# pythoncrazy/jimm

Measured on NVIDIA H100. Metric: images/sec, higher is better.
Workload: dtype f16

## Files before the change

jimm_b200/csrc/common.cuh:

```cuda
#pragma once

#include <cuda.h>
#include <cuda_bf16.h>
#include <cuda_fp16.h>
#include <cuda_runtime.h>
#include <stdint.h>

namespace jimm {

void set_last_error(const char* fmt, ...);

#define JIMM_CUDA_CHECK(expr)                                                                   \
  do {                                                                                          \
    cudaError_t _e = (expr);                                                                    \
    if (_e != cudaSuccess) {                                                                    \
      ::jimm::set_last_error("%s:%d: %s -> %s", __FILE__, __LINE__, #expr, cudaGetErrorString(_e)); \
      return -2;                                                                                \
    }                                                                                           \
  } while (0)

void note_launch();
#define JIMM_LAUNCH_CHECK()                  \
  do {                                       \
    JIMM_CUDA_CHECK(cudaGetLastError());     \
    ::jimm::note_launch();                   \
  } while (0)

int pdl_enabled();
template <typename... KArgs, typename... Args>
inline cudaError_t launch_k(void (*kernel)(KArgs...), dim3 grid, dim3 block, size_t smem, cudaStream_t stream, int cluster_x, bool pdl,
                            Args&&... args) {
  cudaLaunchConfig_t cfg = {};
  cfg.gridDim = grid;
  cfg.blockDim = block;
  cfg.dynamicSmemBytes = smem;
  cfg.stream = stream;
  cudaLaunchAttribute attr[2];
  unsigned n = 0;
  if (pdl && pdl_enabled()) {
    attr[n].id = cudaLaunchAttributeProgrammaticStreamSerialization;
    attr[n].val.programmaticStreamSerializationAllowed = 1;
    ++n;
  }
  if (cluster_x > 1) {
    attr[n].id = cudaLaunchAttributeClusterDimension;
    attr[n].val.clusterDim.x = static_cast<unsigned>(cluster_x);
    attr[n].val.clusterDim.y = 1;
    attr[n].val.clusterDim.z = 1;
    ++n;
  }
  cfg.attrs = attr;
  cfg.numAttrs = n;
  return cudaLaunchKernelEx(&cfg, kernel, static_cast<KArgs>(args)...);
}

struct DeviceOnce {
  static constexpr int kMaxDevices = 64;
  bool done[kMaxDevices] = {};
  bool first() {
    int dev = 0;
    cudaGetDevice(&dev);
    if (dev < 0 || dev >= kMaxDevices) return true;
    if (done[dev]) return false;
    done[dev] = true;
    return true;
  }
};

__device__ __forceinline__ void pdl_launch_dependents() { asm volatile("griddepcontrol.launch_dependents;" ::: "memory"); }
__device__ __forceinline__ void pdl_wait() { asm volatile("griddepcontrol.wait;" ::: "memory"); }

__device__ __forceinline__ uint32_t smem_u32(const void* p) {
  return static_cast<uint32_t>(__cvta_generic_to_shared(p));
}

__device__ __forceinline__ uint32_t lane_id() {
  uint32_t l;
  asm volatile("mov.u32 %0, %%laneid;" : "=r"(l));
  return l;
}

__device__ __forceinline__ bool elect_one_sync() {
  uint32_t pred = 0;
  asm volatile(
      "{\n\t.reg .pred P1;\n\t"
      "elect.sync _|P1, 0xffffffff;\n\t"
      "selp.u32 %0, 1, 0, P1;\n\t}"
      : "=r"(pred));
  return pred != 0;
}

__device__ __forceinline__ void mbar_init(uint64_t* bar, uint32_t count) {
  asm volatile("mbarrier.init.shared::cta.b64 [%0], %1;" ::"r"(smem_u32(bar)), "r"(count));
}
__device__ __forceinline__ void fence_barrier_init() {
  asm volatile("fence.mbarrier_init.release.cluster;" ::: "memory");
}
__device__ __forceinline__ void fence_proxy_async_smem() {
  asm volatile("fence.proxy.async.shared::cta;" ::: "memory");
}
__device__ __forceinline__ void mbar_arrive(uint64_t* bar) {
  asm volatile("mbarrier.arrive.shared::cta.b64 _, [%0];" ::"r"(smem_u32(bar)) : "memory");
}
__device__ __forceinline__ void mbar_arrive_expect_tx(uint64_t* bar, uint32_t bytes) {
  asm volatile("mbarrier.arrive.expect_tx.shared::cta.b64 _, [%0], %1;" ::"r"(smem_u32(bar)), "r"(bytes) : "memory");
}
__device__ __forceinline__ void mbar_wait(uint64_t* bar, uint32_t parity) {
  asm volatile(
      "{\n\t.reg .pred P1;\n\t"
      "WAIT_LOOP:\n\t"
      "mbarrier.try_wait.parity.shared::cta.b64 P1, [%0], %1;\n\t"
      "@P1 bra DONE;\n\t"
      "bra WAIT_LOOP;\n\t"
      "DONE:\n\t}" ::"r"(smem_u32(bar)),
      "r"(parity)
      : "memory");
}

__device__ __forceinline__ bool mbar_test_wait(uint64_t* bar, uint32_t parity) {
  uint32_t ok;
  asm volatile(
      "{\n\t.reg .pred P1;\n\t"
      "mbarrier.test_wait.parity.shared::cta.b64 P1, [%1], %2;\n\t"
      "selp.u32 %0, 1, 0, P1;\n\t}"
      : "=r"(ok)
      : "r"(smem_u32(bar)), "r"(parity)
      : "memory");
  return ok != 0;
}

__device__ __forceinline__ void tma_prefetch_desc(const CUtensorMap* m) {
  asm volatile("prefetch.tensormap [%0];" ::"l"(reinterpret_cast<uint64_t>(m)) : "memory");
}
__device__ __forceinline__ void tma_load_2d(void* smem_dst, const CUtensorMap* m, uint64_t* bar, int c0, int c1) {
  asm volatile(
      "cp.async.bulk.tensor.2d.shared::cluster.global.mbarrier::complete_tx::bytes [%0], [%1, {%3, %4}], [%2];" ::"r"(
          smem_u32(smem_dst)),
      "l"(reinterpret_cast<uint64_t>(m)), "r"(smem_u32(bar)), "r"(c0), "r"(c1)
      : "memory");
}

__device__ __forceinline__ void tma_store_2d(const CUtensorMap* m, uint32_t smem_src, int c0, int c1) {
  asm volatile("cp.async.bulk.tensor.2d.global.shared::cta.bulk_group [%0, {%2, %3}], [%1];" ::"l"(reinterpret_cast<uint64_t>(m)),
               "r"(smem_src), "r"(c0), "r"(c1)
               : "memory");
}
__device__ __forceinline__ void tma_reduce_add_2d(const CUtensorMap* m, uint32_t smem_src, int c0, int c1) {
  asm volatile("cp.reduce.async.bulk.tensor.2d.global.shared::cta.add.tile.bulk_group [%0, {%2, %3}], [%1];" ::"l"(
                   reinterpret_cast<uint64_t>(m)),
               "r"(smem_src), "r"(c0), "r"(c1)
               : "memory");
}
__device__ __forceinline__ void tma_store_3d(const CUtensorMap* m, uint32_t smem_src, int c0, int c1, int c2) {
  asm volatile("cp.async.bulk.tensor.3d.global.shared::cta.bulk_group [%0, {%2, %3, %4}], [%1];" ::"l"(reinterpret_cast<uint64_t>(m)),
               "r"(smem_src), "r"(c0), "r"(c1), "r"(c2)
               : "memory");
}
__device__ __forceinline__ void tma_reduce_add_3d(const CUtensorMap* m, uint32_t smem_src, int c0, int c1, int c2) {
  asm volatile("cp.reduce.async.bulk.tensor.3d.global.shared::cta.add.tile.bulk_group [%0, {%2, %3, %4}], [%1];" ::"l"(
                   reinterpret_cast<uint64_t>(m)),
               "r"(smem_src), "r"(c0), "r"(c1), "r"(c2)
               : "memory");
}
__device__ __forceinline__ void tma_store_commit() { asm volatile("cp.async.bulk.commit_group;" ::: "memory"); }
__device__ __forceinline__ void tma_store_wait_read() { asm volatile("cp.async.bulk.wait_group.read 0;" ::: "memory"); }
__device__ __forceinline__ void tma_store_wait_read1() { asm volatile("cp.async.bulk.wait_group.read 1;" ::: "memory"); }
__device__ __forceinline__ void tma_store_wait_all() { asm volatile("cp.async.bulk.wait_group 0;" ::: "memory"); }

__device__ __forceinline__ uint32_t cluster_ctarank() {
  uint32_t r;
  asm volatile("mov.u32 %0, %%cluster_ctarank;" : "=r"(r));
  return r;
}
__device__ __forceinline__ void cluster_sync_all() {
  asm volatile("barrier.cluster.arrive.release.aligned;\n\tbarrier.cluster.wait.acquire.aligned;" ::: "memory");
}
__device__ __forceinline__ uint32_t mapa_shared(uint32_t local_smem_addr, uint32_t rank) {
  uint32_t r;
  asm volatile("mapa.shared::cluster.u32 %0, %1, %2;" : "=r"(r) : "r"(local_smem_addr), "r"(rank));
  return r;
}
__device__ __forceinline__ void mbar_arrive_cluster(uint32_t cluster_addr) {
  asm volatile("mbarrier.arrive.release.cluster.shared::cluster.b64 _, [%0];" ::"r"(cluster_addr) : "memory");
}
__device__ __forceinline__ uint64_t make_wgmma_desc_sw128(uint32_t smem_addr) {
  uint64_t d = 0;
  d |= static_cast<uint64_t>((smem_addr & 0x3FFFFu) >> 4);
  d |= static_cast<uint64_t>(1) << 16;
  d |= static_cast<uint64_t>(1024 >> 4) << 32;
  d |= static_cast<uint64_t>(1) << 62;
  return d;
}
__device__ __forceinline__ void wgmma_fence() { asm volatile("wgmma.fence.sync.aligned;" ::: "memory"); }
__device__ __forceinline__ void wgmma_commit() { asm volatile("wgmma.commit_group.sync.aligned;" ::: "memory"); }
template <int N>
__device__ __forceinline__ void wgmma_wait() { asm volatile("wgmma.wait_group.sync.aligned %0;" ::"n"(N) : "memory"); }
template <int R>
__device__ __forceinline__ void wgmma_fence_operands(float (&d)[R]) {
#pragma unroll
  for (int i = 0; i < R; ++i) asm volatile("" : "+f"(d[i])::"memory");
}

template <int KIND>
__device__ __forceinline__ void wgmma_m64n128_ss(float (&d)[64], uint64_t adesc, uint64_t bdesc, uint32_t accumulate) {
  if constexpr (KIND == 0) {
    asm volatile(
        "{\n\t.reg .pred p;\n\t"
        "setp.ne.b32 p, %66, 0;\n\t"
        "wgmma.mma_async.sync.aligned.m64n128k16.f32.f16.f16 {%0, %1, %2, %3, %4, %5, %6, %7, %8, %9, %10, %11, %12, %13, %14, %15, %16, %17, %18, %19, %20, %21, %22, %23, %24, %25, %26, %27, %28, %29, %30, %31, %32, %33, %34, %35, %36, %37, %38, %39, %40, %41, %42, %43, %44, %45, %46, %47, %48, %49, %50, %51, %52, %53, %54, %55, %56, %57, %58, %59, %60, %61, %62, %63}, %64, %65, p, 1, 1, 0, 0;\n\t}"
        : "+f"(d[0]), "+f"(d[1]), "+f"(d[2]), "+f"(d[3]), "+f"(d[4]), "+f"(d[5]), "+f"(d[6]), "+f"(d[7]),
          "+f"(d[8]), "+f"(d[9]), "+f"(d[10]), "+f"(d[11]), "+f"(d[12]), "+f"(d[13]), "+f"(d[14]), "+f"(d[15]),
          "+f"(d[16]), "+f"(d[17]), "+f"(d[18]), "+f"(d[19]), "+f"(d[20]), "+f"(d[21]), "+f"(d[22]), "+f"(d[23]),
          "+f"(d[24]), "+f"(d[25]), "+f"(d[26]), "+f"(d[27]), "+f"(d[28]), "+f"(d[29]), "+f"(d[30]), "+f"(d[31]),
          "+f"(d[32]), "+f"(d[33]), "+f"(d[34]), "+f"(d[35]), "+f"(d[36]), "+f"(d[37]), "+f"(d[38]), "+f"(d[39]),
          "+f"(d[40]), "+f"(d[41]), "+f"(d[42]), "+f"(d[43]), "+f"(d[44]), "+f"(d[45]), "+f"(d[46]), "+f"(d[47]),
          "+f"(d[48]), "+f"(d[49]), "+f"(d[50]), "+f"(d[51]), "+f"(d[52]), "+f"(d[53]), "+f"(d[54]), "+f"(d[55]),
          "+f"(d[56]), "+f"(d[57]), "+f"(d[58]), "+f"(d[59]), "+f"(d[60]), "+f"(d[61]), "+f"(d[62]), "+f"(d[63])
        : "l"(adesc), "l"(bdesc), "r"(accumulate));
  } else if constexpr (KIND == 1) {
    asm volatile(
        "{\n\t.reg .pred p;\n\t"
        "setp.ne.b32 p, %66, 0;\n\t"
        "wgmma.mma_async.sync.aligned.m64n128k16.f32.bf16.bf16 {%0, %1, %2, %3, %4, %5, %6, %7, %8, %9, %10, %11, %12, %13, %14, %15, %16, %17, %18, %19, %20, %21, %22, %23, %24, %25, %26, %27, %28, %29, %30, %31, %32, %33, %34, %35, %36, %37, %38, %39, %40, %41, %42, %43, %44, %45, %46, %47, %48, %49, %50, %51, %52, %53, %54, %55, %56, %57, %58, %59, %60, %61, %62, %63}, %64, %65, p, 1, 1, 0, 0;\n\t}"
        : "+f"(d[0]), "+f"(d[1]), "+f"(d[2]), "+f"(d[3]), "+f"(d[4]), "+f"(d[5]), "+f"(d[6]), "+f"(d[7]),
          "+f"(d[8]), "+f"(d[9]), "+f"(d[10]), "+f"(d[11]), "+f"(d[12]), "+f"(d[13]), "+f"(d[14]), "+f"(d[15]),
          "+f"(d[16]), "+f"(d[17]), "+f"(d[18]), "+f"(d[19]), "+f"(d[20]), "+f"(d[21]), "+f"(d[22]), "+f"(d[23]),
          "+f"(d[24]), "+f"(d[25]), "+f"(d[26]), "+f"(d[27]), "+f"(d[28]), "+f"(d[29]), "+f"(d[30]), "+f"(d[31]),
          "+f"(d[32]), "+f"(d[33]), "+f"(d[34]), "+f"(d[35]), "+f"(d[36]), "+f"(d[37]), "+f"(d[38]), "+f"(d[39]),
          "+f"(d[40]), "+f"(d[41]), "+f"(d[42]), "+f"(d[43]), "+f"(d[44]), "+f"(d[45]), "+f"(d[46]), "+f"(d[47]),
          "+f"(d[48]), "+f"(d[49]), "+f"(d[50]), "+f"(d[51]), "+f"(d[52]), "+f"(d[53]), "+f"(d[54]), "+f"(d[55]),
          "+f"(d[56]), "+f"(d[57]), "+f"(d[58]), "+f"(d[59]), "+f"(d[60]), "+f"(d[61]), "+f"(d[62]), "+f"(d[63])
        : "l"(adesc), "l"(bdesc), "r"(accumulate));
  } else {
    asm volatile(
        "{\n\t.reg .pred p;\n\t"
        "setp.ne.b32 p, %66, 0;\n\t"
        "wgmma.mma_async.sync.aligned.m64n128k8.f32.tf32.tf32 {%0, %1, %2, %3, %4, %5, %6, %7, %8, %9, %10, %11, %12, %13, %14, %15, %16, %17, %18, %19, %20, %21, %22, %23, %24, %25, %26, %27, %28, %29, %30, %31, %32, %33, %34, %35, %36, %37, %38, %39, %40, %41, %42, %43, %44, %45, %46, %47, %48, %49, %50, %51, %52, %53, %54, %55, %56, %57, %58, %59, %60, %61, %62, %63}, %64, %65, p, 1, 1;\n\t}"
        : "+f"(d[0]), "+f"(d[1]), "+f"(d[2]), "+f"(d[3]), "+f"(d[4]), "+f"(d[5]), "+f"(d[6]), "+f"(d[7]),
          "+f"(d[8]), "+f"(d[9]), "+f"(d[10]), "+f"(d[11]), "+f"(d[12]), "+f"(d[13]), "+f"(d[14]), "+f"(d[15]),
          "+f"(d[16]), "+f"(d[17]), "+f"(d[18]), "+f"(d[19]), "+f"(d[20]), "+f"(d[21]), "+f"(d[22]), "+f"(d[23]),
          "+f"(d[24]), "+f"(d[25]), "+f"(d[26]), "+f"(d[27]), "+f"(d[28]), "+f"(d[29]), "+f"(d[30]), "+f"(d[31]),
          "+f"(d[32]), "+f"(d[33]), "+f"(d[34]), "+f"(d[35]), "+f"(d[36]), "+f"(d[37]), "+f"(d[38]), "+f"(d[39]),
          "+f"(d[40]), "+f"(d[41]), "+f"(d[42]), "+f"(d[43]), "+f"(d[44]), "+f"(d[45]), "+f"(d[46]), "+f"(d[47]),
          "+f"(d[48]), "+f"(d[49]), "+f"(d[50]), "+f"(d[51]), "+f"(d[52]), "+f"(d[53]), "+f"(d[54]), "+f"(d[55]),
          "+f"(d[56]), "+f"(d[57]), "+f"(d[58]), "+f"(d[59]), "+f"(d[60]), "+f"(d[61]), "+f"(d[62]), "+f"(d[63])
        : "l"(adesc), "l"(bdesc), "r"(accumulate));
  }
}

template <bool BF16>
__device__ __forceinline__ void wgmma_m64n64k16_ss(float (&d)[32], uint64_t adesc, uint64_t bdesc, uint32_t accumulate) {
  if constexpr (BF16) {
    asm volatile(
        "{\n\t.reg .pred p;\n\t"
        "setp.ne.b32 p, %34, 0;\n\t"
        "wgmma.mma_async.sync.aligned.m64n64k16.f32.bf16.bf16 {%0, %1, %2, %3, %4, %5, %6, %7, %8, %9, %10, %11, %12, %13, %14, %15, %16, %17, %18, %19, %20, %21, %22, %23, %24, %25, %26, %27, %28, %29, %30, %31}, %32, %33, p, 1, 1, 0, 0;\n\t}"
        : "+f"(d[0]), "+f"(d[1]), "+f"(d[2]), "+f"(d[3]), "+f"(d[4]), "+f"(d[5]), "+f"(d[6]), "+f"(d[7]),
          "+f"(d[8]), "+f"(d[9]), "+f"(d[10]), "+f"(d[11]), "+f"(d[12]), "+f"(d[13]), "+f"(d[14]), "+f"(d[15]),
          "+f"(d[16]), "+f"(d[17]), "+f"(d[18]), "+f"(d[19]), "+f"(d[20]), "+f"(d[21]), "+f"(d[22]), "+f"(d[23]),
          "+f"(d[24]), "+f"(d[25]), "+f"(d[26]), "+f"(d[27]), "+f"(d[28]), "+f"(d[29]), "+f"(d[30]), "+f"(d[31])
        : "l"(adesc), "l"(bdesc), "r"(accumulate));
  } else {
    asm volatile(
        "{\n\t.reg .pred p;\n\t"
        "setp.ne.b32 p, %34, 0;\n\t"
        "wgmma.mma_async.sync.aligned.m64n64k16.f32.f16.f16 {%0, %1, %2, %3, %4, %5, %6, %7, %8, %9, %10, %11, %12, %13, %14, %15, %16, %17, %18, %19, %20, %21, %22, %23, %24, %25, %26, %27, %28, %29, %30, %31}, %32, %33, p, 1, 1, 0, 0;\n\t}"
        : "+f"(d[0]), "+f"(d[1]), "+f"(d[2]), "+f"(d[3]), "+f"(d[4]), "+f"(d[5]), "+f"(d[6]), "+f"(d[7]),
          "+f"(d[8]), "+f"(d[9]), "+f"(d[10]), "+f"(d[11]), "+f"(d[12]), "+f"(d[13]), "+f"(d[14]), "+f"(d[15]),
          "+f"(d[16]), "+f"(d[17]), "+f"(d[18]), "+f"(d[19]), "+f"(d[20]), "+f"(d[21]), "+f"(d[22]), "+f"(d[23]),
          "+f"(d[24]), "+f"(d[25]), "+f"(d[26]), "+f"(d[27]), "+f"(d[28]), "+f"(d[29]), "+f"(d[30]), "+f"(d[31])
        : "l"(adesc), "l"(bdesc), "r"(accumulate));
  }
}
template <bool BF16>
__device__ __forceinline__ void wgmma_m64n64k16_rs(float (&d)[32], const uint32_t (&a)[4], uint64_t bdesc) {
  if constexpr (BF16) {
    asm volatile(
        "wgmma.mma_async.sync.aligned.m64n64k16.f32.bf16.bf16 {%0, %1, %2, %3, %4, %5, %6, %7, %8, %9, %10, %11, %12, %13, %14, %15, %16, %17, %18, %19, %20, %21, %22, %23, %24, %25, %26, %27, %28, %29, %30, %31}, {%32, %33, %34, %35}, %36, 1, 1, 1, 1;"
        : "+f"(d[0]), "+f"(d[1]), "+f"(d[2]), "+f"(d[3]), "+f"(d[4]), "+f"(d[5]), "+f"(d[6]), "+f"(d[7]),
          "+f"(d[8]), "+f"(d[9]), "+f"(d[10]), "+f"(d[11]), "+f"(d[12]), "+f"(d[13]), "+f"(d[14]), "+f"(d[15]),
          "+f"(d[16]), "+f"(d[17]), "+f"(d[18]), "+f"(d[19]), "+f"(d[20]), "+f"(d[21]), "+f"(d[22]), "+f"(d[23]),
          "+f"(d[24]), "+f"(d[25]), "+f"(d[26]), "+f"(d[27]), "+f"(d[28]), "+f"(d[29]), "+f"(d[30]), "+f"(d[31])
        : "r"(a[0]), "r"(a[1]), "r"(a[2]), "r"(a[3]), "l"(bdesc));
  } else {
    asm volatile(
        "wgmma.mma_async.sync.aligned.m64n64k16.f32.f16.f16 {%0, %1, %2, %3, %4, %5, %6, %7, %8, %9, %10, %11, %12, %13, %14, %15, %16, %17, %18, %19, %20, %21, %22, %23, %24, %25, %26, %27, %28, %29, %30, %31}, {%32, %33, %34, %35}, %36, 1, 1, 1, 1;"
        : "+f"(d[0]), "+f"(d[1]), "+f"(d[2]), "+f"(d[3]), "+f"(d[4]), "+f"(d[5]), "+f"(d[6]), "+f"(d[7]),
          "+f"(d[8]), "+f"(d[9]), "+f"(d[10]), "+f"(d[11]), "+f"(d[12]), "+f"(d[13]), "+f"(d[14]), "+f"(d[15]),
          "+f"(d[16]), "+f"(d[17]), "+f"(d[18]), "+f"(d[19]), "+f"(d[20]), "+f"(d[21]), "+f"(d[22]), "+f"(d[23]),
          "+f"(d[24]), "+f"(d[25]), "+f"(d[26]), "+f"(d[27]), "+f"(d[28]), "+f"(d[29]), "+f"(d[30]), "+f"(d[31])
        : "r"(a[0]), "r"(a[1]), "r"(a[2]), "r"(a[3]), "l"(bdesc));
  }
}

__device__ __forceinline__ void named_bar_sync(int id, int nthreads) { asm volatile("bar.sync %0, %1;" ::"r"(id), "r"(nthreads) : "memory"); }

__device__ __forceinline__ float tanh_fast(float x) {
  float y;
  asm("tanh.approx.f32 %0, %1;" : "=f"(y) : "f"(x));
  return y;
}
__device__ __forceinline__ float ex2_fast(float x) {
  float y;
  asm("ex2.approx.ftz.f32 %0, %1;" : "=f"(y) : "f"(x));
  return y;
}
__device__ __forceinline__ float rcp_fast(float x) {
  float y;
  asm("rcp.approx.ftz.f32 %0, %1;" : "=f"(y) : "f"(x));
  return y;
}
__device__ __forceinline__ float gelu_tanh(float x) {
  const float c0 = -2.0f * 0.7978845608028654f * 1.4426950408889634f;
  const float c1 = c0 * 0.044715f;
  const float z = x * fmaf(x * x, c1, c0);
  return x * rcp_fast(1.0f + ex2_fast(z));
}
__device__ __forceinline__ float quick_gelu(float x) { return x * rcp_fast(1.0f + ex2_fast(x * (-1.702f * 1.4426950408889634f))); }

__device__ __forceinline__ float warp_sum(float v) {
#pragma unroll
  for (int o = 16; o > 0; o >>= 1) v += __shfl_xor_sync(0xffffffffu, v, o);
  return v;
}
__device__ __forceinline__ float warp_max(float v) {
#pragma unroll
  for (int o = 16; o > 0; o >>= 1) v = fmaxf(v, __shfl_xor_sync(0xffffffffu, v, o));
  return v;
}

__device__ __forceinline__ float round_tf32(float v) {
  uint32_t u;
  asm("cvt.rna.tf32.f32 %0, %1;" : "=r"(u) : "f"(v));
  return __uint_as_float(u);
}
struct tf32_t {
  float v;
};

template <typename T>
__device__ __forceinline__ T from_float(float v);
template <>
__device__ __forceinline__ tf32_t from_float<tf32_t>(float v) { return tf32_t{round_tf32(v)}; }
template <>
__device__ __forceinline__ float from_float<float>(float v) { return v; }
template <>
__device__ __forceinline__ __half from_float<__half>(float v) { return __float2half_rn(v); }
template <>
__device__ __forceinline__ __nv_bfloat16 from_float<__nv_bfloat16>(float v) { return __float2bfloat16_rn(v); }

__device__ __forceinline__ float to_float(float v) { return v; }
__device__ __forceinline__ float to_float(__half v) { return __half2float(v); }
__device__ __forceinline__ float to_float(__nv_bfloat16 v) { return __bfloat162float(v); }

__device__ __forceinline__ uint32_t pack2(float a, float b, int out_type ) {
  if (out_type == 1) {
    __half2 h = __floats2half2_rn(a, b);
    return *reinterpret_cast<uint32_t*>(&h);
  } else {
    __nv_bfloat162 h = __floats2bfloat162_rn(a, b);
    return *reinterpret_cast<uint32_t*>(&h);
  }
}

}
```

jimm_b200/csrc/gemm.cu:

```cuda
#include "gemm.cuh"

#include <stdarg.h>
#include <stdio.h>
#include <stdlib.h>
#include <string.h>

#include <type_traits>

#include "common.cuh"

namespace jimm {

static constexpr int BM = 128;
static constexpr int BN = 128;
static constexpr int STAGES = 5;
static constexpr int A_STAGE_BYTES = BM * 128;
static constexpr int B_STAGE_BYTES = BN * 128;
static constexpr int STAGE_BYTES = A_STAGE_BYTES + B_STAGE_BYTES;
static constexpr int EPI_WARPS = 8;
static constexpr int EPI_BOX_ROWS = 16;
static constexpr int EPI_BUF_BYTES = EPI_BOX_ROWS * 128;
static constexpr int EPI_BUFS = 2;
static constexpr int EPI_STAGE_BYTES = EPI_WARPS * EPI_BUFS * EPI_BUF_BYTES;
static constexpr int NUM_THREADS = 384;

enum OutKind : int { OUT_GENERIC = 0, OUT_H16 = 1, OUT_BF16 = 2, OUT_TF32 = 3, OUT_F32_ADD = 4, OUT_F32 = 5 };

struct EpiDev {
  const float* bias;
  const float* rowadd;
  const float* residual;
  void* out;
  int act, ldr, out_type, ldo, rows_in, rows_out, row_off, mode;
  int M, N;
  int reverse;
  int tok_pad, tok_off;
  const float* ln_scale;
  const float* ln_bias;
  void* ln_out;
  int* ln_cnt;
  int ln_out_type, ln_ldo;
  float ln_eps;
};

template <int ACT>
__device__ __forceinline__ float act_ct(float v) {
  if constexpr (ACT == ACT_GELU_TANH) return gelu_tanh(v);
  else if constexpr (ACT == ACT_QUICK_GELU) return quick_gelu(v);
  else return v;
}
__device__ __forceinline__ float apply_act(float v, int act) {
  if (act == ACT_GELU_TANH) return gelu_tanh(v);
  if (act == ACT_QUICK_GELU) return quick_gelu(v);
  return v;
}

__device__ __forceinline__ void remap_row(const EpiDev& e, int row, int& out_row, int& add_row) {
  if (e.rows_in > 0) {
    int b = row / e.rows_in, p = row - b * e.rows_in;
    out_row = b * e.rows_out + p + e.row_off;
    add_row = p + e.row_off;
  } else {
    out_row = row;
    add_row = row;
  }
}

__device__ __forceinline__ void store1(const EpiDev& e, int out_row, int col, float v) {
  size_t off = static_cast<size_t>(out_row) * e.ldo + col;
  if (e.out_type == DT_F32) static_cast<float*>(e.out)[off] = v;
  else if (e.out_type == DT_TF32) static_cast<float*>(e.out)[off] = round_tf32(v);
  else if (e.out_type == DT_F16) static_cast<__half*>(e.out)[off] = __float2half_rn(v);
  else static_cast<__nv_bfloat16*>(e.out)[off] = __float2bfloat16_rn(v);
}

template <typename T>
struct Traits;
template <>
struct Traits<__half> {
  static constexpr int KIND = 0;
};
template <>
struct Traits<__nv_bfloat16> {
  static constexpr int KIND = 1;
};
template <>
struct Traits<float> {
  static constexpr int KIND = 2;
};

static constexpr int ACT_FUSE_LN = 7;
static constexpr int LNQ = 240;
struct LnQueue {
  int head, tail, done, pad;
  int slot[LNQ];
};

template <typename OutT, int NV>
__device__ __forceinline__ void ln_rows_nv(const EpiDev& e, int row0, int lane) {
  constexpr int R0 = 12 / NV;
  constexpr int R = R0 < 1 ? 1 : (R0 > 8 ? 8 : R0);
  constexpr bool DOUBLE = NV <= 9;
  const float inv_d = 1.0f / static_cast<float>(NV * 128);
  const float4* sc = reinterpret_cast<const float4*>(e.ln_scale);
  const float4* bi = reinterpret_cast<const float4*>(e.ln_bias);
  const float* xbase = static_cast<const float*>(e.out);
  const int ldx = e.ldo, ldh = e.ln_ldo;
  const float eps = e.ln_eps;
  OutT* hbase = static_cast<OutT*>(e.ln_out);
  const int rows = min(32, e.M - row0);
  float4 a[R][NV];
  float4 b[DOUBLE ? R : 1][DOUBLE ? NV : 1];
#define JIMM_LN_LOAD(buf, r0_)                                                                                          \
  _Pragma("unroll") for (int i = 0; i < R; ++i) {      \
    const float4* xr = reinterpret_cast<const float4*>(xbase + static_cast<size_t>(row0 + min((r0_) + i, rows - 1)) * ldx); \
    _Pragma("unroll") for (int j = 0; j < NV; ++j) buf[i][j] = __ldcg(xr + lane + 32 * j);                              \
  }
#define JIMM_LN_PROCESS(buf, r0_)                                                                                       \
  _Pragma("unroll") for (int i = 0; i < R; ++i) {                                                                       \
    if ((r0_) + i < rows) {                                                                                             \
      float s = 0.f, s2 = 0.f;                                                                                          \
      _Pragma("unroll") for (int j = 0; j < NV; ++j) {                                                                  \
        const float4 v = buf[i][j];                                                                                     \
        s += v.x + v.y + v.z + v.w;                                                                                     \
        s2 += v.x * v.x + v.y * v.y + v.z * v.z + v.w * v.w;                                                            \
      }                                                                                                                 \
      s = warp_sum(s);                                                                                                  \
      s2 = warp_sum(s2);                                                                                                \
      const float mean = s * inv_d;                                                                                     \
      const float rstd = rsqrtf(fmaxf(s2 * inv_d - mean * mean, 0.0f) + eps);                                           \
      OutT* orow = hbase + static_cast<size_t>(row0 + (r0_) + i) * ldh;                                                 \
      _Pragma("unroll") for (int j = 0; j < NV; ++j) {                                                                  \
        const int idx = lane + 32 * j;                                                                                  \
        const float4 v = buf[i][j], g = __ldg(sc + idx), bb = __ldg(bi + idx);                                          \
        float4 y;                                                                                                       \
        y.x = (v.x - mean) * rstd * g.x + bb.x;                                                                         \
        y.y = (v.y - mean) * rstd * g.y + bb.y;                                                                         \
        y.z = (v.z - mean) * rstd * g.z + bb.z;                                                                         \
        y.w = (v.w - mean) * rstd * g.w + bb.w;                                                                         \
        if constexpr (std::is_same<OutT, float>::value) {                                                               \
          reinterpret_cast<float4*>(orow)[idx] = make_float4(round_tf32(y.x), round_tf32(y.y), round_tf32(y.z), round_tf32(y.w)); \
        } else {                                                                                                        \
          uint2 pk;                                                                                                     \
          constexpr int ot = std::is_same<OutT, __half>::value ? DT_F16 : DT_BF16;                                      \
          pk.x = pack2(y.x, y.y, ot);                                                                                   \
          pk.y = pack2(y.z, y.w, ot);                                                                                   \
          reinterpret_cast<uint2*>(orow)[idx] = pk;                                                                     \
        }                                                                                                               \
      }                                                                                                                 \
    }                                                                                                                   \
  }
  if constexpr (DOUBLE) {
    JIMM_LN_LOAD(a, 0)
#pragma unroll 1
    for (int r0 = 0; r0 < rows; r0 += 2 * R) {
      JIMM_LN_LOAD(b, r0 + R)
      JIMM_LN_PROCESS(a, r0)
      JIMM_LN_LOAD(a, r0 + 2 * R)
      JIMM_LN_PROCESS(b, r0 + R)
    }
  } else {
#pragma unroll 1
    for (int r0 = 0; r0 < rows; r0 += R) {
      JIMM_LN_LOAD(a, r0)
      JIMM_LN_PROCESS(a, r0)
    }
  }
#undef JIMM_LN_LOAD
#undef JIMM_LN_PROCESS
}

template <typename OutT>
__device__ __forceinline__ void ln_rows_dispatch(const EpiDev& e, int row0, int lane) {
  switch (e.N >> 7) {
    case 1: ln_rows_nv<OutT, 1>(e, row0, lane); break;
    case 2: ln_rows_nv<OutT, 2>(e, row0, lane); break;
    case 3: ln_rows_nv<OutT, 3>(e, row0, lane); break;
    case 4: ln_rows_nv<OutT, 4>(e, row0, lane); break;
    case 6: ln_rows_nv<OutT, 6>(e, row0, lane); break;
    case 8: ln_rows_nv<OutT, 8>(e, row0, lane); break;
    case 9: ln_rows_nv<OutT, 9>(e, row0, lane); break;
    case 10: ln_rows_nv<OutT, 10>(e, row0, lane); break;
    case 12: ln_rows_nv<OutT, 12>(e, row0, lane); break;
    default: break;
  }
}

__device__ __forceinline__ void ln_publish(const EpiDev& e, LnQueue* q, int rg, int cols) {
  tma_store_wait_all();
  __threadfence();
  const int old = atomicAdd(e.ln_cnt + rg, cols);
  if (old + cols == 2 * e.N) {
    e.ln_cnt[rg] = 0;
    __threadfence();
    const int t = atomicAdd(&q->tail, 1);
    volatile int* s = &q->slot[t % LNQ];
    while (*s != -1) __nanosleep(64);
    *s = rg;
  }
}

template <typename OutT>
__device__ __forceinline__ void ln_worker(const EpiDev& e, LnQueue* q, int lane) {
  for (;;) {
    int rg = -2;
    if (lane == 0) {
      const int t = atomicAdd(&q->head, 1);
      volatile int* s = &q->slot[t % LNQ];
      for (;;) {
        if (*s >= 0) {
          const int v = atomicExch(&q->slot[t % LNQ], -1);
          if (v >= 0) { rg = v; break; }
        }
        if (*reinterpret_cast<volatile int*>(&q->done) == EPI_WARPS && t >= *reinterpret_cast<volatile int*>(&q->tail)) break;
        __nanosleep(256);
      }
      __threadfence();
    }
    rg = __shfl_sync(0xffffffffu, rg, 0);
    if (rg < 0) return;
    ln_rows_dispatch<OutT>(e, rg * 32, lane);
  }
}

template <int OUT, int ACT>
__device__ __forceinline__ void epilogue_tma(const CUtensorMap* map_c, const EpiDev& epi, const float (&acc)[64], uint8_t* tbuf0, int lane,
                                             int row_base, int n_tile0, uint32_t& box_count) {
  constexpr bool OUT16 = (OUT == OUT_H16 || OUT == OUT_BF16);
  constexpr int ES = OUT16 ? 2 : 4;
  constexpr int COLS_PER_BOX = 128 / ES;
  constexpr int JB = COLS_PER_BOX / 8;
  const int g = lane >> 2, t = lane & 3;
#pragma unroll
  for (int s = 0; s < BN / COLS_PER_BOX; ++s) {
    const int n0 = n_tile0 + s * COLS_PER_BOX;
    if (n0 >= epi.N) break;
    uint8_t* tbuf = tbuf0 + (box_count & (EPI_BUFS - 1)) * EPI_BUF_BYTES;
    ++box_count;
    if (lane == 0) tma_store_wait_read1();
    __syncwarp();
#pragma unroll
    for (int jj = 0; jj < JB; ++jj) {
      const int j = s * JB + jj;
      const int col = n0 + jj * 8 + 2 * t;
      float2 b2 = make_float2(0.f, 0.f);
      if (epi.bias != nullptr && col < epi.N) b2 = __ldg(reinterpret_cast<const float2*>(epi.bias + col));
      const float v0 = act_ct<ACT>(acc[4 * j] + b2.x), v1 = act_ct<ACT>(acc[4 * j + 1] + b2.y);
      const float v2 = act_ct<ACT>(acc[4 * j + 2] + b2.x), v3 = act_ct<ACT>(acc[4 * j + 3] + b2.y);
      const int byte = (jj * 8 + 2 * t) * ES;
      const int off = ((((byte >> 4) ^ g)) << 4) + (byte & 15);
      uint8_t* p0 = tbuf + g * 128 + off;
      uint8_t* p1 = p0 + 8 * 128;
      if constexpr (OUT16) {
        *reinterpret_cast<uint32_t*>(p0) = pack2(v0, v1, OUT == OUT_H16 ? 1 : 2);
        *reinterpret_cast<uint32_t*>(p1) = pack2(v2, v3, OUT == OUT_H16 ? 1 : 2);
      } else if constexpr (OUT == OUT_TF32) {
        *reinterpret_cast<float2*>(p0) = make_float2(round_tf32(v0), round_tf32(v1));
        *reinterpret_cast<float2*>(p1) = make_float2(round_tf32(v2), round_tf32(v3));
      } else {
        *reinterpret_cast<float2*>(p0) = make_float2(v0, v1);
        *reinterpret_cast<float2*>(p1) = make_float2(v2, v3);
      }
    }
    fence_proxy_async_smem();
    __syncwarp();
    if (lane == 0) {
      const uint32_t tbuf_u32 = smem_u32(tbuf);
      if constexpr (OUT == OUT_F32_ADD) {
        if (epi.tok_pad > 0) {
          const int b = row_base / epi.tok_pad;
          tma_reduce_add_3d(map_c, tbuf_u32, n0, row_base - b * epi.tok_pad + epi.tok_off, b);
        } else {
          tma_reduce_add_2d(map_c, tbuf_u32, n0, row_base);
        }
      } else {
        tma_store_2d(map_c, tbuf_u32, n0, row_base);
      }
      tma_store_commit();
    }
  }
}

__device__ __forceinline__ void epilogue_generic(const EpiDev& epi, const float (&acc)[64], int lane, int row_base, int n_tile0) {
  const int g = lane >> 2, t = lane & 3;
#pragma unroll
  for (int h = 0; h < 2; ++h) {
    const int row = row_base + g + 8 * h;
    if (row >= epi.M) continue;
    int out_row, add_row;
    remap_row(epi, row, out_row, add_row);
#pragma unroll
    for (int j = 0; j < BN / 8; ++j) {
#pragma unroll
      for (int q = 0; q < 2; ++q) {
        const int col = n_tile0 + 8 * j + 2 * t + q;
        if (col < epi.N) {
          float v = acc[4 * j + 2 * h + q];
          if (epi.bias) v += __ldg(epi.bias + col);
          v = apply_act(v, epi.act);
          if (epi.rowadd) v += __ldg(epi.rowadd + static_cast<size_t>(add_row) * epi.N + col);
          if (epi.residual) v += epi.residual[static_cast<size_t>(out_row) * epi.ldr + col];
          store1(epi, out_row, col, v);
        }
      }
    }
  }
}

template <typename T, int OUT, int ACT>
__global__ void __launch_bounds__(NUM_THREADS, 1)
gemm_wgmma_kernel(const __grid_constant__ CUtensorMap map_a, const __grid_constant__ CUtensorMap map_b,
                  const __grid_constant__ CUtensorMap map_c, const EpiDev epi, int K) {
  constexpr int BK = 128 / sizeof(T);
  constexpr int UK = 32 / sizeof(T);
  constexpr bool FUSE_LN = OUT == OUT_F32_ADD && ACT == ACT_FUSE_LN;
  constexpr int EPI_ACT = ACT == ACT_FUSE_LN ? static_cast<int>(ACT_NONE) : ACT;

  extern __shared__ uint8_t smem_raw[];
  uint8_t* smem = reinterpret_cast<uint8_t*>((reinterpret_cast<uintptr_t>(smem_raw) + 1023) & ~static_cast<uintptr_t>(1023));
  uint8_t* smem_a = smem;
  uint8_t* smem_b = smem + STAGES * A_STAGE_BYTES;
  uint8_t* epi_stage = smem + STAGES * STAGE_BYTES;
  LnQueue* lnq = reinterpret_cast<LnQueue*>(epi_stage + EPI_STAGE_BYTES);
  uint64_t* full_bar = reinterpret_cast<uint64_t*>(lnq + 1);
  uint64_t* empty_bar = full_bar + STAGES;

  const int warp_idx = threadIdx.x >> 5;
  const int lane = threadIdx.x & 31;
  const int M = epi.M, N = epi.N;
  const int m_tiles = (M + BM - 1) / BM, n_tiles = (N + BN - 1) / BN;
  const int num_tiles = m_tiles * n_tiles;
  const int num_kb = (K + BK - 1) / BK;

  pdl_launch_dependents();
  if (warp_idx == 0 && lane == 0) {
    tma_prefetch_desc(&map_a);
    tma_prefetch_desc(&map_b);
    if constexpr (OUT != OUT_GENERIC) tma_prefetch_desc(&map_c);
    for (int s = 0; s < STAGES; ++s) {
      mbar_init(&full_bar[s], 1);
      mbar_init(&empty_bar[s], EPI_WARPS);
    }
    fence_barrier_init();
  }
  if constexpr (FUSE_LN) {
    if (warp_idx == 1) {
      for (int i = lane; i < LNQ; i += 32) lnq->slot[i] = -1;
      if (lane == 0) lnq->head = lnq->tail = lnq->done = 0;
    }
  }
  __syncthreads();
  pdl_wait();

  if (warp_idx < 4) {
    if (warp_idx == 0) {
      if (lane == 0) {
        int stage = 0;
        uint32_t phase = 0;
        for (int tile = blockIdx.x; tile < num_tiles; tile += gridDim.x) {
          const int tv = epi.reverse ? num_tiles - 1 - tile : tile;
          const int m_blk = tv / n_tiles, n_blk = tv - m_blk * n_tiles;
          for (int kb = 0; kb < num_kb; ++kb) {
            mbar_wait(&empty_bar[stage], phase ^ 1);
            mbar_arrive_expect_tx(&full_bar[stage], STAGE_BYTES);
            tma_load_2d(smem_a + stage * A_STAGE_BYTES, &map_a, &full_bar[stage], kb * BK, m_blk * BM);
            tma_load_2d(smem_b + stage * B_STAGE_BYTES, &map_b, &full_bar[stage], kb * BK, n_blk * BN);
            if (++stage == STAGES) { stage = 0; phase ^= 1; }
          }
        }
      }
    } else if constexpr (FUSE_LN) {
      ln_worker<T>(epi, lnq, lane);
    }
  } else {
    const int wg = (warp_idx - 4) >> 2;
    const int wq = warp_idx & 3;
    uint8_t* tbuf0 = epi_stage + (warp_idx - 4) * EPI_BUFS * EPI_BUF_BYTES;
    int stage = 0;
    uint32_t phase = 0, box_count = 0;
    int ln_rg = -1, ln_cols = 0;
    float acc[64];
    for (int tile = blockIdx.x; tile < num_tiles; tile += gridDim.x) {
      const int tv = epi.reverse ? num_tiles - 1 - tile : tile;
      const int m_blk = tv / n_tiles, n_blk = tv - m_blk * n_tiles;
      int prev = -1;
      for (int kb = 0; kb < num_kb; ++kb) {
        mbar_wait(&full_bar[stage], phase);
        const uint64_t adesc = make_wgmma_desc_sw128(smem_u32(smem_a + stage * A_STAGE_BYTES + wg * 64 * 128));
        const uint64_t bdesc = make_wgmma_desc_sw128(smem_u32(smem_b + stage * B_STAGE_BYTES));
        wgmma_fence_operands(acc);
        wgmma_fence();
#pragma unroll
        for (int k = 0; k < BK / UK; ++k)
          wgmma_m64n128_ss<Traits<T>::KIND>(acc, adesc + static_cast<uint64_t>(2 * k), bdesc + static_cast<uint64_t>(2 * k), (kb | k) != 0 ? 1u : 0u);
        wgmma_commit();
        wgmma_fence_operands(acc);
        if (prev >= 0) {
          wgmma_wait<1>();
          if (lane == 0) mbar_arrive(&empty_bar[prev]);
        }
        prev = stage;
        if (++stage == STAGES) { stage = 0; phase ^= 1; }
      }
      wgmma_wait<0>();
      wgmma_fence_operands(acc);
      if (lane == 0) mbar_arrive(&empty_bar[prev]);

      const int row_base = m_blk * BM + wg * 64 + wq * 16;
      const int n_tile0 = n_blk * BN;
      if constexpr (OUT == OUT_GENERIC) {
        epilogue_generic(epi, acc, lane, row_base, n_tile0);
      } else {
        if (row_base < M) epilogue_tma<OUT, EPI_ACT>(&map_c, epi, acc, tbuf0, lane, row_base, n_tile0, box_count);
        if constexpr (FUSE_LN) {
          if (lane == 0 && ln_rg >= 0) ln_publish(epi, lnq, ln_rg, ln_cols);
          ln_rg = (row_base & ~31) < M ? row_base >> 5 : -1;
          ln_cols = min(BN, N - n_tile0);
        }
      }
    }
    if constexpr (FUSE_LN) {
      if (lane == 0) {
        if (ln_rg >= 0) ln_publish(epi, lnq, ln_rg, ln_cols);
        __threadfence_block();
        atomicAdd(&lnq->done, 1);
      }
    }
    if constexpr (OUT != OUT_GENERIC) {
      if (lane == 0) tma_store_wait_all();
    }
  }
}

template <typename T>
__global__ void gemm_simt_kernel(const T* __restrict__ A, int lda, const T* __restrict__ B, int ldb, int K, EpiDev epi) {
  __shared__ float As[16][17], Bs[16][17];
  const int tx = threadIdx.x, ty = threadIdx.y;
  const int row = blockIdx.y * 16 + ty, col = blockIdx.x * 16 + tx;
  float acc = 0.f;
  for (int k0 = 0; k0 < K; k0 += 16) {
    const int ar = blockIdx.y * 16 + ty, ak = k0 + tx;
    As[ty][tx] = (ar < epi.M && ak < K) ? to_float(A[static_cast<size_t>(ar) * lda + ak]) : 0.f;
    const int br = blockIdx.x * 16 + ty, bk = k0 + tx;
    Bs[ty][tx] = (br < epi.N && bk < K) ? to_float(B[static_cast<size_t>(br) * ldb + bk]) : 0.f;
    __syncthreads();
#pragma unroll
    for (int k = 0; k < 16; ++k) acc += As[ty][k] * Bs[tx][k];
    __syncthreads();
  }
  if (row < epi.M && col < epi.N) {
    int out_row, add_row;
    remap_row(epi, row, out_row, add_row);
    float v = acc;
    if (epi.bias) v += epi.bias[col];
    v = apply_act(v, epi.act);
    if (epi.rowadd) v += epi.rowadd[static_cast<size_t>(add_row) * epi.N + col];
    if (epi.residual) v += epi.residual[static_cast<size_t>(out_row) * epi.ldr + col];
    store1(epi, out_row, col, v);
  }
}

static constexpr int SMEM_BYTES = STAGES * STAGE_BYTES + EPI_STAGE_BYTES + static_cast<int>(sizeof(LnQueue)) + 2 * STAGES * 8 + 1024;
static_assert(SMEM_BYTES <= 232448, "exceeds 227 KB of shared memory");
typedef CUresult (*PFN_encodeTiled)(CUtensorMap*, CUtensorMapDataType, cuuint32_t, void*, const cuuint64_t*, const cuuint64_t*,
                                    const cuuint32_t*, const cuuint32_t*, CUtensorMapInterleave, CUtensorMapSwizzle,
                                    CUtensorMapL2promotion, CUtensorMapFloatOOBfill);

static PFN_encodeTiled get_encode_fn() {
  static PFN_encodeTiled fn = nullptr;
  if (fn) return fn;
  void* p = nullptr;
  cudaDriverEntryPointQueryResult qres;
  cudaError_t e = cudaGetDriverEntryPoint("cuTensorMapEncodeTiled", &p, cudaEnableDefault, &qres);
  if (e != cudaSuccess || qres != cudaDriverEntryPointSuccess || p == nullptr) {
    set_last_error("cudaGetDriverEntryPoint(cuTensorMapEncodeTiled) failed: %s", cudaGetErrorString(e));
    return nullptr;
  }
  fn = reinterpret_cast<PFN_encodeTiled>(p);
  return fn;
}

static int make_map(CUtensorMap* map, int dtype, const void* ptr, int rows, int K, int ld, int box_rows) {
  PFN_encodeTiled enc = get_encode_fn();
  if (!enc) return -3;
  const size_t es = dtype_size(dtype);
  CUtensorMapDataType dt = (dtype == DT_F32 || dtype == DT_TF32) ? CU_TENSOR_MAP_DATA_TYPE_FLOAT32
                                           : (dtype == DT_F16 ? CU_TENSOR_MAP_DATA_TYPE_FLOAT16 : CU_TENSOR_MAP_DATA_TYPE_BFLOAT16);
  cuuint64_t dims[2] = {static_cast<cuuint64_t>(K), static_cast<cuuint64_t>(rows)};
  cuuint64_t strides[1] = {static_cast<cuuint64_t>(ld) * es};
  cuuint32_t box[2] = {static_cast<cuuint32_t>(128 / es), static_cast<cuuint32_t>(box_rows)};
  cuuint32_t estr[2] = {1, 1};
  if ((reinterpret_cast<uintptr_t>(ptr) & 15) != 0 || (strides[0] & 15) != 0) {
    set_last_error("gemm: operand pointer/stride must be 16-byte aligned (ptr=%p, ld=%d)", ptr, ld);
    return -1;
  }
  CUresult r = enc(map, dt, 2, const_cast<void*>(ptr), dims, strides, box, estr, CU_TENSOR_MAP_INTERLEAVE_NONE,
                   CU_TENSOR_MAP_SWIZZLE_128B, CU_TENSOR_MAP_L2_PROMOTION_L2_256B, CU_TENSOR_MAP_FLOAT_OOB_FILL_NONE);
  if (r != CUDA_SUCCESS) {
    set_last_error("cuTensorMapEncodeTiled failed: CUresult %d (rows=%d K=%d ld=%d)", static_cast<int>(r), rows, K, ld);
    return -3;
  }
  return 0;
}

int make_tensor_map_3d(CUtensorMap* map, int dtype, const void* ptr, int B, int S, int N, int ld) {
  PFN_encodeTiled enc = get_encode_fn();
  if (!enc) return -3;
  const size_t es = dtype_size(dtype);
  CUtensorMapDataType dt = (dtype == DT_F32 || dtype == DT_TF32) ? CU_TENSOR_MAP_DATA_TYPE_FLOAT32
                                           : (dtype == DT_F16 ? CU_TENSOR_MAP_DATA_TYPE_FLOAT16 : CU_TENSOR_MAP_DATA_TYPE_BFLOAT16);
  cuuint64_t dims[3] = {static_cast<cuuint64_t>(N), static_cast<cuuint64_t>(S), static_cast<cuuint64_t>(B)};
  cuuint64_t strides[2] = {static_cast<cuuint64_t>(ld) * es, static_cast<cuuint64_t>(S) * ld * es};
  cuuint32_t box[3] = {static_cast<cuuint32_t>(128 / es), EPI_BOX_ROWS, 1};
  cuuint32_t estr[3] = {1, 1, 1};
  CUresult r = enc(map, dt, 3, const_cast<void*>(ptr), dims, strides, box, estr, CU_TENSOR_MAP_INTERLEAVE_NONE,
                   CU_TENSOR_MAP_SWIZZLE_128B, CU_TENSOR_MAP_L2_PROMOTION_L2_256B, CU_TENSOR_MAP_FLOAT_OOB_FILL_NONE);
  if (r != CUDA_SUCCESS) { set_last_error("cuTensorMapEncodeTiled(3d) failed: CUresult %d", static_cast<int>(r)); return -3; }
  return 0;
}
static int make_map_3d_f32(CUtensorMap* map, const void* ptr, int B, int S, int N, int ld) { return make_tensor_map_3d(map, DT_F32, ptr, B, S, N, ld); }

int make_tensor_map_2d(CUtensorMap* map, int dtype, const void* ptr, int rows, int cols, int ld, int box_rows) {
  return make_map(map, dtype, ptr, rows, cols, ld, box_rows);
}

int device_sm_count() {
  static int sms[DeviceOnce::kMaxDevices] = {};
  int dev = 0;
  cudaGetDevice(&dev);
  if (dev < 0 || dev >= DeviceOnce::kMaxDevices) dev = 0;
  if (sms[dev] == 0) {
    int n = 0;
    cudaDeviceGetAttribute(&n, cudaDevAttrMultiProcessorCount, dev);
    const char* env = getenv("JIMM_NUM_SMS");
    if (env && atoi(env) > 0) n = atoi(env);
    sms[dev] = n;
  }
  return sms[dev];
}

static int check_epi(const GemmEpilogue& e, int N) {
  if (e.out == nullptr) { set_last_error("gemm: null output"); return -1; }
  if (e.ldo < N) { set_last_error("gemm: ldo (%d) < N (%d)", e.ldo, N); return -1; }
  return 0;
}
int gemm_plan_init(GemmPlan* plan, int dtype, const void* A, int lda, const void* B, int ldb, int M, int N, int K,
                   const GemmEpilogue& epi) {
  if (M <= 0 || N <= 0 || K <= 0) { set_last_error("gemm: bad shape %dx%dx%d", M, N, K); return -1; }
  if (int rc = check_epi(epi, N)) return rc;
  if (int rc = make_map(&plan->map_a, dtype, A, M, K, lda, BM)) return rc;
  if (int rc = make_map(&plan->map_b, dtype, B, N, K, ldb, BN)) return rc;
  plan->M = M; plan->N = N; plan->K = K; plan->dtype = dtype; plan->epi = epi;
  memset(&plan->map_c, 0, sizeof(plan->map_c));
  if (plan->epi.mode == 2) {
    const size_t es = dtype_size(epi.out_type);
    const bool ok = epi.rowadd == nullptr && epi.rows_in == 0 &&
                    (epi.residual == nullptr || (epi.residual == epi.out && epi.ldr == epi.ldo && epi.out_type == DT_F32)) &&
                    (static_cast<size_t>(epi.ldo) * es) % 16 == 0 && (reinterpret_cast<uintptr_t>(epi.out) & 15) == 0 &&
                    (epi.bias == nullptr || ((reinterpret_cast<uintptr_t>(epi.bias) & 15) == 0 && N % 4 == 0)) &&
                    !(epi.residual && epi.act != ACT_NONE);
    if (ok && epi.tok_pad > 0) {
      if (epi.tok_pad % EPI_BOX_ROWS != 0 || M % epi.tok_pad != 0 || !epi.residual) { set_last_error("gemm: bad token-scatter epilogue"); return -1; }
      if (int rc = make_map_3d_f32(&plan->map_c, epi.out, M / epi.tok_pad, epi.tok_S, N, epi.ldo)) return rc;
    } else if (ok) {
      if (int rc = make_map(&plan->map_c, epi.out_type, epi.out, M, N, epi.ldo, EPI_BOX_ROWS)) return rc;
    } else {
      plan->epi.mode = 0;
    }
  }
  return 0;
}

static EpiDev to_dev(const GemmEpilogue& e, int M, int N) {
  EpiDev d;
  d.bias = e.bias; d.rowadd = e.rowadd; d.residual = e.residual; d.out = e.out;
  d.act = e.act; d.ldr = e.ldr; d.out_type = e.out_type; d.ldo = e.ldo;
  d.rows_in = e.rows_in; d.rows_out = e.rows_out; d.row_off = e.row_off; d.mode = e.mode;
  d.M = M; d.N = N;
  d.tok_pad = e.tok_pad; d.tok_off = e.tok_off;
  d.reverse = e.reverse;
  d.ln_scale = e.ln_scale; d.ln_bias = e.ln_bias; d.ln_out = e.ln_out; d.ln_cnt = e.ln_cnt;
  d.ln_out_type = e.ln_out_type; d.ln_ldo = e.ln_ldo; d.ln_eps = e.ln_eps;
  return d;
}

template <typename T, int OUT, int ACT>
static int launch_one(const GemmPlan* p, int M, cudaStream_t stream) {
  static DeviceOnce attr_set;
  if (attr_set.first()) JIMM_CUDA_CHECK(cudaFuncSetAttribute(gemm_wgmma_kernel<T, OUT, ACT>, cudaFuncAttributeMaxDynamicSharedMemorySize, SMEM_BYTES));
  const int tiles = ((M + BM - 1) / BM) * ((p->N + BN - 1) / BN);
  const int grid = tiles < device_sm_count() ? tiles : device_sm_count();
  JIMM_CUDA_CHECK(launch_k(gemm_wgmma_kernel<T, OUT, ACT>, dim3(grid), dim3(NUM_THREADS), SMEM_BYTES, stream, 1, true, p->map_a, p->map_b,
                           p->map_c, to_dev(p->epi, M, p->N), p->K));
  note_launch();
  return 0;
}

template <typename T, int OUT>
static int launch_act(const GemmPlan* p, int M, cudaStream_t stream) {
  switch (p->epi.act) {
    case ACT_GELU_TANH: return launch_one<T, OUT, ACT_GELU_TANH>(p, M, stream);
    case ACT_QUICK_GELU: return launch_one<T, OUT, ACT_QUICK_GELU>(p, M, stream);
    default: return launch_one<T, OUT, ACT_NONE>(p, M, stream);
  }
}

template <typename T>
static int launch_tc(const GemmPlan* p, int M, cudaStream_t stream) {
  const GemmEpilogue& e = p->epi;
  if (e.mode != 2) return launch_one<T, OUT_GENERIC, ACT_NONE>(p, M, stream);
  if (e.residual) return gemm_fuses_ln(p, M) ? launch_one<T, OUT_F32_ADD, ACT_FUSE_LN>(p, M, stream) : launch_one<T, OUT_F32_ADD, ACT_NONE>(p, M, stream);
  switch (e.out_type) {
    case DT_F16: return launch_act<T, OUT_H16>(p, M, stream);
    case DT_BF16: return launch_act<T, OUT_BF16>(p, M, stream);
    case DT_TF32: return launch_act<T, OUT_TF32>(p, M, stream);
    default: return launch_act<T, OUT_F32>(p, M, stream);
  }
}

int gemm_fuses_ln(const GemmPlan* p, int ) {
  const int nv = p->N >> 7;
  const bool width_ok = p->N % 128 == 0 && (nv <= 4 || nv == 6 || (nv >= 8 && nv <= 10) || nv == 12);
  const int want = p->dtype == DT_F16 ? DT_F16 : p->dtype == DT_BF16 ? DT_BF16 : DT_TF32;
  return p->epi.ln_cnt != nullptr && p->epi.ln_out_type == want && width_ok && p->epi.mode == 2 && p->epi.residual != nullptr && p->epi.tok_pad == 0;
}

int gemm_plan_run(const GemmPlan* p0, int M_override, cudaStream_t stream, int reverse) {
  const int M = (M_override > 0 && M_override <= p0->M) ? M_override : p0->M;
  GemmPlan local;
  const GemmPlan* p = p0;
  if (reverse != p0->epi.reverse) { local = *p0; local.epi.reverse = reverse; p = &local; }
  switch (p->dtype) {
    case DT_F16: return launch_tc<__half>(p, M, stream);
    case DT_BF16: return launch_tc<__nv_bfloat16>(p, M, stream);
    case DT_F32:
    case DT_TF32: return launch_tc<float>(p, M, stream);
  }
  set_last_error("gemm: bad dtype %d", p->dtype);
  return -1;
}

int gemm_simt_run(int dtype, const void* A, int lda, const void* B, int ldb, int M, int N, int K, const GemmEpilogue& epi,
                  cudaStream_t stream) {
  if (int rc = check_epi(epi, N)) return rc;
  dim3 block(16, 16), grid((N + 15) / 16, (M + 15) / 16);
  EpiDev d = to_dev(epi, M, N);
  if (dtype == DT_F16) gemm_simt_kernel<__half><<<grid, block, 0, stream>>>(static_cast<const __half*>(A), lda, static_cast<const __half*>(B), ldb, K, d);
  else if (dtype == DT_BF16) gemm_simt_kernel<__nv_bfloat16><<<grid, block, 0, stream>>>(static_cast<const __nv_bfloat16*>(A), lda, static_cast<const __nv_bfloat16*>(B), ldb, K, d);
  else gemm_simt_kernel<float><<<grid, block, 0, stream>>>(static_cast<const float*>(A), lda, static_cast<const float*>(B), ldb, K, d);
  JIMM_LAUNCH_CHECK();
  return 0;
}

}
```

Baseline: 11530.

## Ping-pong consumer warpgroups over whole tiles with register reallocation

Each consumer warpgroup now computes a full 128x128 tile, using two 64-row accumulators, and the two warpgroups alternate tiles. Named barriers order their mainloops so one warpgroup's epilogue overlaps the other's MMA. setmaxnreg moves registers from the producer warps to the consumer warps to hold the doubled accumulators, and the LN worker's row batching is reduced to fit its smaller register budget. The empty barrier count becomes 4 because only one warpgroup consumes each stage. This risks register spills and serialization between the warpgroups, and it lowers LN throughput.

```diff
diff --git a/jimm_b200/csrc/common.cuh b/jimm_b200/csrc/common.cuh
--- a/jimm_b200/csrc/common.cuh
+++ b/jimm_b200/csrc/common.cuh
@@ -294,6 +294,12 @@
 }
 
 __device__ __forceinline__ void named_bar_sync(int id, int nthreads) { asm volatile("bar.sync %0, %1;" ::"r"(id), "r"(nthreads) : "memory"); }
+__device__ __forceinline__ void named_bar_arrive(int id, int nthreads) { asm volatile("bar.arrive %0, %1;" ::"r"(id), "r"(nthreads) : "memory"); }
+
+template <int N>
+__device__ __forceinline__ void setmaxnreg_dec() { asm volatile("setmaxnreg.dec.sync.aligned.u32 %0;" ::"n"(N)); }
+template <int N>
+__device__ __forceinline__ void setmaxnreg_inc() { asm volatile("setmaxnreg.inc.sync.aligned.u32 %0;" ::"n"(N)); }
 
 __device__ __forceinline__ float tanh_fast(float x) {
   float y;
diff --git a/jimm_b200/csrc/gemm.cu b/jimm_b200/csrc/gemm.cu
--- a/jimm_b200/csrc/gemm.cu
+++ b/jimm_b200/csrc/gemm.cu
@@ -23,6 +23,10 @@
 static constexpr int EPI_BUFS = 2;
 static constexpr int EPI_STAGE_BYTES = EPI_WARPS * EPI_BUFS * EPI_BUF_BYTES;
 static constexpr int NUM_THREADS = 384;
+static constexpr int PRODUCER_REGS = 40, CONSUMER_REGS = 232;
+static constexpr int PRODUCER_REGS_LN = 152, CONSUMER_REGS_LN = 176;
+static_assert(PRODUCER_REGS + 2 * CONSUMER_REGS <= 3 * 168 && PRODUCER_REGS_LN + 2 * CONSUMER_REGS_LN <= 3 * 168, "register pool");
+static constexpr int ORDER_BAR = 1;
 
 enum OutKind : int { OUT_GENERIC = 0, OUT_H16 = 1, OUT_BF16 = 2, OUT_TF32 = 3, OUT_F32_ADD = 4, OUT_F32 = 5 };
 
@@ -98,9 +102,9 @@
 
 template <typename OutT, int NV>
 __device__ __forceinline__ void ln_rows_nv(const EpiDev& e, int row0, int lane) {
-  constexpr int R0 = 12 / NV;
-  constexpr int R = R0 < 1 ? 1 : (R0 > 8 ? 8 : R0);
-  constexpr bool DOUBLE = NV <= 9;
+  constexpr int R0 = 6 / NV;
+  constexpr int R = R0 < 1 ? 1 : R0;
+  constexpr bool DOUBLE = NV <= 6;
   const float inv_d = 1.0f / static_cast<float>(NV * 128);
   const float4* sc = reinterpret_cast<const float4*>(e.ln_scale);
   const float4* bi = reinterpret_cast<const float4*>(e.ln_bias);
@@ -339,7 +343,7 @@
     if constexpr (OUT != OUT_GENERIC) tma_prefetch_desc(&map_c);
     for (int s = 0; s < STAGES; ++s) {
       mbar_init(&full_bar[s], 1);
-      mbar_init(&empty_bar[s], EPI_WARPS);
+      mbar_init(&empty_bar[s], 4);
     }
     fence_barrier_init();
   }
@@ -353,6 +357,7 @@
   pdl_wait();
 
   if (warp_idx < 4) {
+    setmaxnreg_dec<FUSE_LN ? PRODUCER_REGS_LN : PRODUCER_REGS>();
     if (warp_idx == 0) {
       if (lane == 0) {
         int stage = 0;
@@ -373,28 +378,40 @@
       ln_worker<T>(epi, lnq, lane);
     }
   } else {
+    setmaxnreg_inc<FUSE_LN ? CONSUMER_REGS_LN : CONSUMER_REGS>();
     const int wg = (warp_idx - 4) >> 2;
     const int wq = warp_idx & 3;
     uint8_t* tbuf0 = epi_stage + (warp_idx - 4) * EPI_BUFS * EPI_BUF_BYTES;
-    int stage = 0;
-    uint32_t phase = 0, box_count = 0;
-    int ln_rg = -1, ln_cols = 0;
-    float acc[64];
-    for (int tile = blockIdx.x; tile < num_tiles; tile += gridDim.x) {
+    const int cta_tiles = (num_tiles - static_cast<int>(blockIdx.x) + static_cast<int>(gridDim.x) - 1) / static_cast<int>(gridDim.x);
+    uint32_t box_count = 0;
+    int ln_rg[2] = {-1, -1}, ln_cols = 0;
+    float acc[2][64];
+    for (int i = wg; i < cta_tiles; i += 2) {
+      const int tile = blockIdx.x + i * gridDim.x;
       const int tv = epi.reverse ? num_tiles - 1 - tile : tile;
       const int m_blk = tv / n_tiles, n_blk = tv - m_blk * n_tiles;
+      const uint32_t slot0 = static_cast<uint32_t>(i) * static_cast<uint32_t>(num_kb);
+      int stage = static_cast<int>(slot0 % STAGES);
+      uint32_t phase = (slot0 / STAGES) & 1;
+      if (i > 0) named_bar_sync(ORDER_BAR + wg, 256);
       int prev = -1;
       for (int kb = 0; kb < num_kb; ++kb) {
         mbar_wait(&full_bar[stage], phase);
-        const uint64_t adesc = make_wgmma_desc_sw128(smem_u32(smem_a + stage * A_STAGE_BYTES + wg * 64 * 128));
+        const uint64_t adesc = make_wgmma_desc_sw128(smem_u32(smem_a + stage * A_STAGE_BYTES));
         const uint64_t bdesc = make_wgmma_desc_sw128(smem_u32(smem_b + stage * B_STAGE_BYTES));
-        wgmma_fence_operands(acc);
+        wgmma_fence_operands(acc[0]);
+        wgmma_fence_operands(acc[1]);
         wgmma_fence();
 #pragma unroll
-        for (int k = 0; k < BK / UK; ++k)
-          wgmma_m64n128_ss<Traits<T>::KIND>(acc, adesc + static_cast<uint64_t>(2 * k), bdesc + static_cast<uint64_t>(2 * k), (kb | k) != 0 ? 1u : 0u);
+        for (int k = 0; k < BK / UK; ++k) {
+          const uint32_t accumulate = (kb | k) != 0 ? 1u : 0u;
+          wgmma_m64n128_ss<Traits<T>::KIND>(acc[0], adesc + static_cast<uint64_t>(2 * k), bdesc + static_cast<uint64_t>(2 * k), accumulate);
+          wgmma_m64n128_ss<Traits<T>::KIND>(acc[1], adesc + static_cast<uint64_t>((64 * 128 >> 4) + 2 * k), bdesc + static_cast<uint64_t>(2 * k),
+                                            accumulate);
+        }
         wgmma_commit();
-        wgmma_fence_operands(acc);
+        wgmma_fence_operands(acc[0]);
+        wgmma_fence_operands(acc[1]);
         if (prev >= 0) {
           wgmma_wait<1>();
           if (lane == 0) mbar_arrive(&empty_bar[prev]);
@@ -402,26 +419,38 @@
         prev = stage;
         if (++stage == STAGES) { stage = 0; phase ^= 1; }
       }
+      if (i + 1 < cta_tiles) named_bar_arrive(ORDER_BAR + (wg ^ 1), 256);
       wgmma_wait<0>();
-      wgmma_fence_operands(acc);
+      wgmma_fence_operands(acc[0]);
+      wgmma_fence_operands(acc[1]);
       if (lane == 0) mbar_arrive(&empty_bar[prev]);
 
-      const int row_base = m_blk * BM + wg * 64 + wq * 16;
       const int n_tile0 = n_blk * BN;
-      if constexpr (OUT == OUT_GENERIC) {
-        epilogue_generic(epi, acc, lane, row_base, n_tile0);
-      } else {
-        if (row_base < M) epilogue_tma<OUT, EPI_ACT>(&map_c, epi, acc, tbuf0, lane, row_base, n_tile0, box_count);
-        if constexpr (FUSE_LN) {
-          if (lane == 0 && ln_rg >= 0) ln_publish(epi, lnq, ln_rg, ln_cols);
-          ln_rg = (row_base & ~31) < M ? row_base >> 5 : -1;
-          ln_cols = min(BN, N - n_tile0);
-        }
+#pragma unroll
+      for (int h = 0; h < 2; ++h) {
+        const int row_base = m_blk * BM + h * 64 + wq * 16;
+        if constexpr (OUT == OUT_GENERIC) {
+          epilogue_generic(epi, acc[h], lane, row_base, n_tile0);
+        } else {
+          if (row_base < M) epilogue_tma<OUT, EPI_ACT>(&map_c, epi, acc[h], tbuf0, lane, row_base, n_tile0, box_count);
+        }
+      }
+      if constexpr (FUSE_LN) {
+        if (lane == 0) {
+          for (int h = 0; h < 2; ++h)
+            if (ln_rg[h] >= 0) ln_publish(epi, lnq, ln_rg[h], ln_cols);
+        }
+        for (int h = 0; h < 2; ++h) {
+          const int row_base = m_blk * BM + h * 64 + wq * 16;
+          ln_rg[h] = (row_base & ~31) < M ? row_base >> 5 : -1;
+        }
+        ln_cols = min(BN, N - n_tile0);
       }
     }
     if constexpr (FUSE_LN) {
       if (lane == 0) {
-        if (ln_rg >= 0) ln_publish(epi, lnq, ln_rg, ln_cols);
+        for (int h = 0; h < 2; ++h)
+          if (ln_rg[h] >= 0) ln_publish(epi, lnq, ln_rg[h], ln_cols);
         __threadfence_block();
         atomicAdd(&lnq->done, 1);
       }
```

New measurement: 11830, median of 6. 1.03x the previous value.
